# JosephCatrambone/aruco3

Hardware: AMD Instinct MI355X
Metric: frames/sec at 1920x1080 ARUCO dict (higher is better)
Workload: dtype u8

## Files before the change

aruco3_amd/_lib.py:

```python
import ctypes as C
from pathlib import Path

import numpy as np

import os

_HERE = Path(__file__).resolve().parent
LIB_PATH = Path(os.environ["A3_HIP_LIB"]).resolve() if os.environ.get("A3_HIP_LIB") else _HERE / "libaruco3_hip.so"

OK, ERR_INVALID, ERR_HIP, ERR_CAPACITY, ERR_INTERNAL, ERR_NO_DEVICE, ERR_LIMIT = 0, -1, -2, -3, -4, -5, -6
FMT_RGB8, FMT_RGBA8, FMT_L8, FMT_BGRA8 = 0, 1, 2, 3
MEM_HOST, MEM_DEVICE = 0, 1
PROFILE_OFF, PROFILE_STAGES, PROFILE_THRESHOLD_ONLY, PROFILE_THRESHOLD_SAMPLED = 0, 1, 2, 3
STAGE_THRESHOLD, STAGE_CONTOUR, STAGE_DECODE = 0, 1, 2
STEP_WHOLE, STEP_DECODE_DEFERRED, STEP_HELD_RELEASED_BY_LAST, STEP_HELD_RELEASED_EARLY, STEP_BURST_LAST, STEP_HELD = 0, 1, 2, 3, 4, 5
REFINE_NONE, REFINE_SUBPIX = 0, 1
BOARD_NONE, BOARD_OK = 0, 1
BOARD_MAX_MARKERS = 1024
DIST_NONE, DIST_RATIONAL = 0, 1
CHARUCO_MAX_CORNERS = 2048
CHARUCO_NO_ADJ = 0xFFFFFFFF
CALIB_FIX_PRINCIPAL_POINT, CALIB_ZERO_TANGENT_DIST, CALIB_FIX_K3, CALIB_RATIONAL_MODEL, CALIB_USE_INTRINSIC_GUESS = 1, 2, 4, 8, 16
CALIB_OK, CALIB_TOO_FEW, CALIB_NO_INIT, CALIB_NOT_FINITE = 1, 2, 3, 4
CALIB_VIEW_USED, CALIB_VIEW_TOO_FEW_POINTS, CALIB_VIEW_DEGENERATE = 1, 2, 3
CALIB_MAX_POINTS, CALIB_MAX_VIEWS, CALIB_MAX_CAMERAS, CALIB_MAX_CALL_VIEWS = 4096, 4096, 1024, 65536
RIG_USE_EXTRINSIC_GUESS, RIG_FIX_EXTRINSICS = 1, 2
RIG_OK, RIG_NOT_CONNECTED, RIG_NOT_FINITE = 1, 2, 3
RIG_OBS_USED, RIG_OBS_TOO_FEW_POINTS, RIG_OBS_DEGENERATE = 1, 2, 3
RIG_FRAME_USED, RIG_FRAME_UNUSED = 1, 2
RIG_MAX_CAMERAS, RIG_MAX_FRAMES, RIG_MAX_RIGS, RIG_MAX_CALL_FRAMES, RIG_MAX_CALL_OBSERVATIONS = 8, 4096, 1024, 65536, 262144
STEP_NAMES = {0: "whole", 1: "decode_deferred", 2: "held_released_by_last", 3: "held_released_early", 4: "burst_last", 5: "held"}

SYMBOLS = [
    "a3_abi_version", "a3_default_config", "a3_create", "a3_destroy", "a3_last_error", "a3_set_stream", "a3_get_stream", "a3_set_pool_limits",
    "a3_get_tau", "a3_order_after", "a3_set_debug_taps", "a3_detect_batch", "a3_detect_batch_pose", "a3_detect_batch_submit", "a3_detect_batch_collect", "a3_detect_batch_pose_submit", "a3_detect_batch_pose_collect",
    "a3_host_alloc", "a3_host_free", "a3_host_register", "a3_host_unregister", "a3_get_stats", "a3_synth_render", "a3_download_grey", "a3_download_thresholded",
    "a3_candidate_count", "a3_download_candidates", "a3_download_homographies", "a3_estimate_pose", "a3_estimate_pose_normalized",
    "a3_find_nearest", "a3_calculate_tau", "a3_set_profiling", "a3_get_profile",
    "a3_contour_count", "a3_download_contours", "a3_detection_record_bytes", "a3_pack_detections",
    "a3_default_refine_config", "a3_set_corner_refinement", "a3_get_refined_corners", "a3_refine_corners",
    "a3_set_board", "a3_get_board_poses", "a3_estimate_board_pose",
    "a3_default_distortion", "a3_set_distortion", "a3_get_undistorted_corners", "a3_undistort_points",
    "a3_default_charuco_config", "a3_set_charuco", "a3_get_charuco_corners", "a3_get_charuco_poses", "a3_interpolate_charuco",
    "a3_calibrate_cameras", "a3_calibrate_rigs",
]
INTERNAL_SYMBOLS = ["a3_debug_set_overlap", "a3_debug_build_flags", "a3_debug_spin", "a3_debug_set_hold", "a3_debug_set_jump_rounds", "a3_debug_launch_threshold", "a3_debug_kernel_time", "a3_selftest_ieee", "a3_debug_clockwise", "a3_debug_rotate_bits", "a3_debug_discard_too_near", "a3_debug_inject_candidates"]


class A3Error(RuntimeError):
    def __init__(self, code, message):
        super().__init__(f"aruco3_hip error {code}: {message}")
        self.code = code


class Config(C.Structure):
    _fields_ = [
        ("threshold_window", C.c_uint32),
        ("contour_simplification_epsilon", C.c_double),
        ("min_side_length_factor", C.c_float),
        ("min_corner_separation_factor", C.c_float),
        ("homography_sample_size", C.c_uint32),
        ("filter_high_bit_errors", C.c_uint8),
    ]


class MarkerRec(C.Structure):
    _fields_ = [
        ("frame", C.c_uint32),
        ("id", C.c_uint32),
# ... 206 lines not shown
    L.a3_download_homographies.argtypes = [vp, C.c_uint32, u8p, u8p, u64p, C.POINTER(C.c_int32), C.c_size_t]
    L.a3_estimate_pose.restype = C.c_int
    L.a3_estimate_pose.argtypes = [vp, u32p, C.c_size_t, C.c_float, C.POINTER(Intrinsics), C.c_uint32, C.c_uint32, C.POINTER(PoseRec)]
    L.a3_estimate_pose_normalized.restype = C.c_int
    L.a3_estimate_pose_normalized.argtypes = [vp, f32p, C.c_size_t, C.c_float, C.POINTER(PoseRec)]
    L.a3_find_nearest.restype = C.c_int
    L.a3_find_nearest.argtypes = [vp, u64p, C.c_size_t, u32p, u8p]
    L.a3_calculate_tau.restype = C.c_int
    L.a3_calculate_tau.argtypes = [C.c_int, u64p, C.c_size_t, u8p]
    L.a3_set_profiling.restype = C.c_int
    L.a3_set_profiling.argtypes = [vp, C.c_int]
    L.a3_get_profile.restype = C.c_int
    L.a3_get_profile.argtypes = [vp, C.c_int, f64p, u64p, C.c_int]
    L.a3_selftest_ieee.restype = C.c_int
    L.a3_selftest_ieee.argtypes = [vp, f64p, f64p, C.c_size_t, f64p, f64p, f32p, f32p]
    L.a3_contour_count.restype = C.c_int
    L.a3_contour_count.argtypes = [vp, C.c_uint32, u32p, u64p]
    L.a3_download_contours.restype = C.c_int
    L.a3_download_contours.argtypes = [vp, C.c_uint32, u32p, u32p, u32p, C.c_size_t, C.c_size_t]
    L.a3_detection_record_bytes.restype = C.c_size_t
    L.a3_detection_record_bytes.argtypes = [C.c_uint32, C.c_int]
    L.a3_pack_detections.restype = C.c_int
    L.a3_pack_detections.argtypes = [vp, C.c_uint32, C.c_uint32, C.c_int, vp, C.c_size_t]
    L.a3_debug_clockwise.restype = C.c_int
    L.a3_debug_clockwise.argtypes = [vp, C.POINTER(C.c_int32), C.c_size_t, C.POINTER(C.c_int32)]
    L.a3_debug_rotate_bits.restype = C.c_int
    L.a3_debug_rotate_bits.argtypes = [vp, u8p, C.c_uint32, C.c_uint32, u8p]
    L.a3_debug_inject_candidates.restype = C.c_int
    L.a3_debug_inject_candidates.argtypes = [vp, u32p, C.c_size_t]
    if hasattr(L, "a3_refine_corners"):
        L.a3_default_refine_config.restype = None
        L.a3_default_refine_config.argtypes = [C.POINTER(RefineConfig)]
        L.a3_set_corner_refinement.restype = C.c_int
        L.a3_set_corner_refinement.argtypes = [vp, C.POINTER(RefineConfig)]
        L.a3_get_refined_corners.restype = C.c_int
        L.a3_get_refined_corners.argtypes = [vp, f32p, C.c_size_t, C.POINTER(C.c_size_t)]
        L.a3_refine_corners.restype = C.c_int
        L.a3_refine_corners.argtypes = [vp, vp, C.c_int, C.c_int, C.c_uint32, C.c_uint32, C.c_size_t, f32p, f32p, C.c_size_t]
    if hasattr(L, "a3_set_board"):
        L.a3_set_board.restype = C.c_int
        L.a3_set_board.argtypes = [vp, u32p, f32p, C.c_size_t]
        L.a3_get_board_poses.restype = C.c_int
        L.a3_get_board_poses.argtypes = [vp, vp, C.c_size_t, C.POINTER(C.c_size_t)]
        L.a3_estimate_board_pose.restype = C.c_int
        L.a3_estimate_board_pose.argtypes = [vp, u32p, f32p, C.c_size_t, C.POINTER(Intrinsics), C.c_uint32, C.c_uint32, C.POINTER(BoardPoseRec)]
    if hasattr(L, "a3_set_distortion"):
# ... 146 lines not shown

    def order_after(self, other: "Context"):
        check(load().a3_order_after(self.handle, other.handle), self.handle)

    def set_debug_taps(self, on: bool):
        check(load().a3_set_debug_taps(self.handle, int(on)), self.handle)

    def set_pool_limits(self, max_darts: int = 0, max_points: int = 0):
        check(load().a3_set_pool_limits(self.handle, max_darts, max_points), self.handle)

    def set_profiling(self, mode):
        check(load().a3_set_profiling(self.handle, int(mode)), self.handle)

    def profile(self, stage: int, reset: bool = False):
        ms, n = C.c_double(), C.c_uint64()
        check(load().a3_get_profile(self.handle, stage, C.byref(ms), C.byref(n), int(reset)), self.handle)
        return float(ms.value), int(n.value)

    def debug_kernel_time(self, kernel: int, dbg: int = 0, reps: int = 5) -> float:
        ms = C.c_float()
        check(load().a3_debug_kernel_time(self.handle, kernel, dbg, reps, C.byref(ms)), self.handle)
        return ms.value

    def stats(self) -> dict:
        s = Stats()
        check(load().a3_get_stats(self.handle, C.byref(s)), self.handle)
        return s.as_dict()

    def detect_batch(self, pixels_ptr: int, memory: int, fmt: int, width: int, height: int, row_stride: int, frame_stride: int, n_frames: int,
                     out_cap: int = 0):
        cap = out_cap or max(64 * n_frames, 64)
        out = np.empty(cap, dtype=MARKER_DTYPE)
        per = np.zeros(max(n_frames, 1), dtype=np.uint32)
        n = C.c_size_t()
        rc = load().a3_detect_batch(self.handle, C.c_void_p(pixels_ptr), memory, fmt, width, height, row_stride, frame_stride, n_frames,
                                    out.ctypes.data_as(C.c_void_p), cap, _p(per, C.c_uint32), C.byref(n))
        check(rc, self.handle)
        return out[: n.value], per[:n_frames]

    def submit(self, pixels_ptr: int, memory: int, fmt: int, width: int, height: int, row_stride: int, frame_stride: int, n_frames: int,
               out_cap: int = 0):
        self._pending = (out_cap or max(64 * n_frames, 64), n_frames)
        check(load().a3_detect_batch_submit(self.handle, C.c_void_p(pixels_ptr), memory, fmt, width, height, row_stride, frame_stride, n_frames,
                                            self._pending[0]), self.handle)

    def collect(self):
# ... 304 lines not shown
```

aruco3_amd/csrc/a3_api.hip:

```cpp
#include <algorithm>
#include <atomic>
#include <cmath>
#include <chrono>
#include <cstddef>
#include <cstdio>
#include <cstring>
#include <mutex>
#include <string>
#include <vector>

#include "a3_common.h"
#include "a3_internal.h"

namespace a3 {
hipError_t launch_grey_threshold(hipStream_t, const uint8_t*, int, size_t, size_t, int, int, uint32_t, uint32_t, uint8_t*, uint64_t*, uint16_t*);
bool threshold_writes_grey_plane(uint32_t radius, const uint8_t* pixels, size_t row_stride, size_t frame_stride, int W);
hipError_t launch_dart_count(hipStream_t, const uint64_t*, int, int, uint32_t, uint32_t, unsigned long long*, uint32_t*, uint64_t, uint32_t*, uint32_t*, void*, size_t);
size_t tile_darts_bytes(uint32_t W, uint32_t H, uint32_t n_frames);
size_t tile_off_offset(uint32_t W, uint32_t H, uint32_t n_frames);
size_t tile_mask_offset_bytes(uint32_t W, uint32_t H, uint32_t n_frames);
hipError_t launch_dart_build(hipStream_t, const uint64_t*, int, int, uint32_t, uint32_t, const uint32_t*, const uint32_t*, uint32_t*, const uint32_t*,
                             uint64_t*, uint32_t*, uint32_t, const uint32_t*, int, const unsigned long long*);
hipError_t launch_zero(hipStream_t, void*, size_t);
size_t entry_state_bytes();
bool finalize_inline(bool frame_entries, bool trust_natural);
size_t fin_state_bytes();
size_t entry_slots(uint32_t);
size_t leader_list_bytes(uint32_t);
hipError_t launch_rank_cycles(hipStream_t, uint32_t, int, const uint64_t*, const uint32_t*,
                              uint32_t*, unsigned int*, void*, void*, void*, uint32_t*, unsigned int*, int, DeviceCounters*, const uint32_t*, int,
                              const uint32_t*, uint32_t*, uint32_t, int, uint32_t, unsigned int*, int);
hipError_t launch_resolve(hipStream_t, const void*, uint32_t, int, const uint64_t*, const uint32_t*, const unsigned int*, uint64_t*, uint64_t*,
                          DeviceCounters*, int, const uint32_t*);
hipError_t launch_select_scatter(hipStream_t, const void*, uint32_t, const uint32_t*, const unsigned int*, const uint32_t*, const uint64_t*,
                                 const uint32_t*, uint32_t, uint32_t,
                                 uint32_t, double, double, ContourRec*, uint32_t*, uint32_t, uint64_t, DeviceCounters*,
                                 const uint64_t*, uint32_t*, const uint32_t*, int, uint32_t*, int, const void*);
hipError_t launch_debug_clockwise(hipStream_t, const int32_t*, uint32_t, int32_t*);
hipError_t launch_unpack_bits(hipStream_t, const uint64_t*, int, int, uint8_t*);
hipError_t launch_contour_quads(hipStream_t, const ContourRec*, const DeviceCounters*, uint32_t, const uint32_t*, double, uint32_t, uint32_t,
                                uint32_t, CandRec*, uint32_t*, unsigned int*, int, uint32_t);
size_t decode_out_bytes();
hipError_t launch_frame_candidates(hipStream_t, const CandRec*, const uint32_t*, uint32_t, uint32_t, float, uint16_t*, uint16_t*, uint32_t*,
                                   uint32_t*, unsigned int*, uint32_t, void*, float*);
uint32_t frame_cand_lds_slots();
// ... 712 lines not shown
    unsigned int* d_leader_count = ctx->scratch_u32 + 16;
    unsigned int* d_dead_count = ctx->scratch_u32 + 48;

    const uint64_t* d_bin = ctx->bin.as<uint64_t>();
    const double image_diag = std::sqrt((double)W * W + (double)H * H);
    const double eps_factor = ctx->cfg.contour_simplification_epsilon;
    const int resolve_iters = ctx->resolve_full_ttl > 0 ? ctx->resolve_iters_hint : 0;
    const int inline_resolve_W = ctx->resolve_full_ttl > 0 ? 0 : (int)W;
    const int keep_all = b.taps ? 1 : 0;
    int rounds_max = 0;
    for (size_t ci = 0; ci < chunks.size(); ci++) {
        const Chunk& c = chunks[ci];
        DeviceCounters* ctr = ctx->counters + ci;
        const uint32_t* fb = ctx->frame_base.as<uint32_t>() + ci * (max_chunk_frames + 1);
        const uint32_t nd = (uint32_t)c.darts;
        if (nd == 0) continue;
        if (ci > 0) {
            A3_HIP(hipMemsetAsync(d_leader_count, 0, 4 * 32, st));
            A3_HIP(hipMemsetAsync(ctx->frame_cursor, 0, (size_t)c.count * 4, st));
        }
        const uint32_t* tile_off = ctx->tile_darts.as<uint32_t>() + tile_off_offset(W, H, n);
        A3_HIP(launch_dart_build(st, d_bin, (int)W, (int)H, c.first, c.count, fb, tile_off, ctx->pix_base.as<uint32_t>(),
                                 ctx->tile_darts.as<uint32_t>(), ctx->d_xy.as<uint64_t>(), ctx->d_succ.as<uint32_t>(), nd, n_live, 0,
                                 reinterpret_cast<const unsigned long long*>(ctx->tile_darts.as<uint8_t>() + tile_mask_offset_bytes(W, H, n))));
        int rounds = 1;
        while ((1ull << rounds) < (uint64_t)c.max_frame_darts && rounds < 31) rounds++;
        rounds += 1;
        rounds = std::min(rounds, ctx->jump_rounds_hint);
        if (const int cap = g_jump_rounds_cap.load(std::memory_order_relaxed); cap > 0 && ctx->jump_rounds_hint < 32) rounds = std::min(rounds, cap);
        rounds_max = std::max(rounds_max, rounds);
        uint32_t* const frame_entries = ctx->entry_global_ttl > 0 ? nullptr : ctx->frame_cursor;
        const bool dense_graph = (uint64_t)nd * 10u >= (uint64_t)c.count * npx;
        unsigned int* const dead_ctr = (keep_all || !dense_graph) ? nullptr : d_dead_count;
        A3_HIP(launch_rank_cycles(st, nd, (int)W, ctx->d_xy.as<uint64_t>(), ctx->d_succ.as<uint32_t>(),
                                  ctx->entry_list.as<uint32_t>(), d_entry_count, ctx->es_a.p, ctx->es_b.p,
                                  ctx->fin.p, ctx->leader_list.as<uint32_t>(), d_leader_count, rounds, ctr, n_live, 0, fb,
                                  frame_entries, c.count, 1, min_edge_length, dead_ctr, inline_resolve_W > 0 ? 1 : 0));
        if (rel_mode == 2) { if (int rc = release_waiting()) return rc; }
        ctx->dbg_nd = nd; ctx->dbg_frames = c.count; ctx->dbg_chunks = (uint32_t)chunks.size();
        A3_HIP(launch_rank_cycles(st, nd, (int)W, ctx->d_xy.as<uint64_t>(), ctx->d_succ.as<uint32_t>(),
                                  ctx->entry_list.as<uint32_t>(), d_entry_count, ctx->es_a.p, ctx->es_b.p,
                                  ctx->fin.p , ctx->leader_list.as<uint32_t>(), d_leader_count, rounds, ctr,
                                  n_live, 0, fb, frame_entries, c.count, 2, min_edge_length, dead_ctr, inline_resolve_W > 0 ? 1 : 0));
        const void* fin = ctx->fin.p;
        A3_HIP(launch_resolve(st, fin, nd, (int)W, ctx->d_xy.as<uint64_t>(), ctx->leader_list.as<uint32_t>(), d_leader_count,
                              ctx->t_cur.as<uint64_t>(), ctx->t_next.as<uint64_t>(), ctr, resolve_iters, n_live));
        A3_HIP(launch_select_scatter(st, fin, nd, ctx->leader_list.as<uint32_t>(), d_leader_count, ctx->d_succ.as<uint32_t>(), ctx->t_cur.as<uint64_t>(), fb,
// ... 666 lines not shown
    if (int rcs_ = need_stream(ctx)) return rcs_;
    hipStream_t st = ctx->stream;
    struct EventPair {
        hipEvent_t e0 = nullptr, e1 = nullptr;
        ~EventPair() { if (e0) (void)hipEventDestroy(e0); if (e1) (void)hipEventDestroy(e1); }
    } evp;
    A3_HIP(hipEventCreate(&evp.e0)); A3_HIP(hipEventCreate(&evp.e1));
    const hipEvent_t e0 = evp.e0, e1 = evp.e1;
    double total = 0.0;
    unsigned int* d_entry_count = ctx->scratch_u32 + 32;
    unsigned int* d_leader_count = ctx->scratch_u32 + 16;
    for (int r = 0; r < reps; r++) {
        A3_HIP(hipMemsetAsync(d_leader_count, 0, 4 * 32, st));
        A3_HIP(hipEventRecord(e0, st));
        if (kernel == 0) {
            A3_HIP(hipMemsetAsync(ctx->frame_darts.p, 0, (size_t)ctx->frames * 8, st));
            A3_HIP(launch_dart_count(st, ctx->bin.as<uint64_t>(), (int)ctx->W, (int)ctx->H, 0, ctx->frames, ctx->frame_darts.as<unsigned long long>(),
                                     ctx->tile_darts.as<uint32_t>(), 0, nullptr, nullptr, nullptr, 0));
        } else if (kernel == 1) {
            A3_HIP(launch_dart_build(st, ctx->bin.as<uint64_t>(), (int)ctx->W, (int)ctx->H, 0, ctx->dbg_frames, ctx->frame_base.as<uint32_t>(),
                                     ctx->tile_darts.as<uint32_t>() + tile_off_offset(ctx->W, ctx->H, ctx->frames), ctx->pix_base.as<uint32_t>(),
                                     ctx->tile_darts.as<uint32_t>(), ctx->d_xy.as<uint64_t>(),
                                     ctx->d_succ.as<uint32_t>(), ctx->dbg_nd, nullptr, dbg ? dbg : 5,
                                     reinterpret_cast<const unsigned long long*>(ctx->tile_darts.as<uint8_t>() + tile_mask_offset_bytes(ctx->W, ctx->H, ctx->frames))));
        } else if (kernel == 2) {
            A3_HIP(launch_rank_cycles(st, ctx->dbg_nd, (int)ctx->W, ctx->d_xy.as<uint64_t>(), ctx->d_succ.as<uint32_t>(),
                                      ctx->entry_list.as<uint32_t>(),
                                      d_entry_count, ctx->es_a.p, ctx->es_b.p, ctx->fin.p,
                                      ctx->leader_list.as<uint32_t>(), d_leader_count, 0, ctx->counters, nullptr, dbg ? dbg : 11, ctx->frame_base.as<uint32_t>(), nullptr, ctx->dbg_frames, 0,
                                      0u, nullptr, 0));
        } else if (kernel == 3 || kernel == 4) {
            if (kernel == 4) {
                const size_t sweep = std::min<size_t>(ctx->pix_base.cap & ~(size_t)15, (size_t)512 << 20);
                if (sweep) A3_HIP(launch_zero(st, ctx->pix_base.p, sweep));
                A3_HIP(hipEventRecord(e0, st));
            }
            A3_HIP(launch_decode(st, ctx->dbg_src, (int)ctx->W, (int)ctx->H, 0, ctx->fin_xy.as<uint16_t>(), ctx->work.as<uint32_t>(), ctx->scratch_u32,
                                 ctx->max_cand, ctx->cfg.homography_sample_size, ctx->mark_size, ctx->cfg.homography_sample_size, ctx->dict.as<uint64_t>(),
                                 ctx->n_codes, ctx->tau, ctx->cfg.filter_high_bit_errors, ctx->proj.p, ctx->wtab.as<float>(), ctx->outs.p, nullptr, 0u, nullptr, 4096,
                                 dbg == 0 ? -1000 : dbg, ctx->frames <= 64u ? 1 : 0));
        } else return fail(ctx, A3_ERR_INVALID, "kernel: 0 dart_count, 1 dart_assign, 2 local_contract, 3 decode, 4 decode on cold frames");
        A3_HIP(hipEventRecord(e1, st));
        A3_HIP(hipStreamSynchronize(st));
        float ms = 0;
        A3_HIP(hipEventElapsedTime(&ms, e0, e1));
        total += ms;
    }
    *avg_ms = (float)(total / reps);
    return A3_OK;
}

int a3_debug_set_overlap(int mode) {
    if (mode < -1 || mode > 2) return A3_ERR_INVALID;
    std::lock_guard<std::mutex> lk(g_defer_mu);
    if (!g_held.empty() || !g_deferred.empty()) return A3_ERR_INVALID;
    g_overlap_force.store(mode, std::memory_order_relaxed);
    return A3_OK;
}

int a3_debug_spin(void* hip_stream, int workgroups, int threads, int usec) {
    if (workgroups < 1 || workgroups > 1024 || threads < 64 || threads > 512 || threads % 64 || usec < 1 || usec > 100000) return A3_ERR_INVALID;
    static uint32_t* sink = nullptr;
    static std::mutex mu;
    {
        std::lock_guard<std::mutex> lk(mu);
        if (!sink) {
            if (hipMalloc(&sink, 4096 * 4) != hipSuccess) return A3_ERR_HIP;
            if (hipMemset(sink, 0, 4096 * 4) != hipSuccess) return A3_ERR_HIP;
        }
    }
    return launch_spin(reinterpret_cast<hipStream_t>(hip_stream), workgroups, threads, usec, sink) == hipSuccess ? A3_OK : A3_ERR_HIP;
// ... 903 lines not shown
```

aruco3_amd/csrc/a3_internal.h:

```cpp
#ifndef ARUCO3_HIP_INTERNAL_H
#define ARUCO3_HIP_INTERNAL_H

#include "../../include/aruco3_hip.h"

#ifdef __cplusplus
extern "C" {
#endif

int  a3_debug_kernel_time(a3_ctx *ctx, int kernel, int dbg, int reps, float *avg_ms);

int  a3_debug_set_overlap(int mode);

int  a3_debug_spin(void *hip_stream, int workgroups, int threads, int usec);

int  a3_debug_set_hold(int on);

int  a3_debug_set_jump_rounds(int rounds);

int  a3_debug_launch_threshold(a3_ctx *ctx, const void *pixels_device, int fmt, uint32_t width, uint32_t height, uint32_t n_frames);

int  a3_debug_build_flags(void);

int  a3_selftest_ieee(a3_ctx *ctx, const double *a, const double *b, size_t n, double *sqrt_a, double *a_div_b,
                      float *sqrtf_a, float *a_divf_b);

int  a3_debug_clockwise(a3_ctx *ctx, const int32_t *quads_xy, size_t n, int32_t *out_xy);
int  a3_debug_rotate_bits(a3_ctx *ctx, const uint8_t *bits, uint32_t n, uint32_t times, uint8_t *out);
int  a3_debug_inject_candidates(a3_ctx *ctx, const uint32_t *quads_xy, size_t n);
int  a3_debug_discard_too_near(a3_ctx *ctx, const uint32_t *quads_xy, size_t n, float min_distance, uint32_t *out_xy, size_t *n_out);

#ifdef __cplusplus
}
// ... 3 lines not shown
```

aruco3_amd/csrc/k_contours.hip:

```cpp
#include <algorithm>

#include "a3_common.h"


namespace a3 {

constexpr int kFinB = 8;
constexpr int kScatB = 1;

struct Nb8 { uint64_t c; uint64_t n[8]; };

__device__ __forceinline__ uint64_t ldw(const uint64_t* __restrict__ img, int wpr, int H, int j, int y) {
    return (y >= 0 && y < H && j >= 0 && j < wpr) ? img[(size_t)y * wpr + j] : 0ull;
}

__device__ __forceinline__ void pdart_words(const Nb8& nb, uint64_t p[8]) {
#pragma unroll
    for (int k = 0; k < 8; k++) {
        uint64_t m = nb.c & nb.n[k] & ~nb.n[(k + 7) & 7];
        if ((k & 1) == 0) m &= ~nb.n[(k + 6) & 7];
        p[k] = m;
    }
}

// ... 289 lines not shown
struct PixLut { uint16_t v[256]; };
constexpr PixLut make_pix_lut() {
    PixLut t{};
    for (uint32_t F = 0; F < 256; F++) {
        const uint32_t rot1 = ((F << 1) | (F >> 7)) & 0xFFu, rot2 = ((F << 2) | (F >> 6)) & 0xFFu;
        const uint32_t P = F & ~rot1 & (0xAAu | ~rot2) & 0xFFu;
        uint32_t kW = 15, kE = 15;
        if (!(F & 1u)) { kW = 0; for (uint32_t b = 0; b < 7; b++) if ((F >> 1) & (1u << b)) { kW = b + 1; break; } }
        if (!(F & 16u)) {
            const uint32_t rr = ((F >> 5) | (F << 3)) & 0xFFu;
            uint32_t first = 0;
            for (uint32_t b = 0; b < 8; b++) if (rr & (1u << b)) { first = b + 1; break; }
            kE = (5 + first - 1) & 7;
        }
        t.v[F] = (uint16_t)(P | (kW << 8) | (kE << 12));
    }
    return t;
}
__device__ __constant__ const PixLut kPixLut = make_pix_lut();

__device__ __forceinline__ int dir_dx(int k) { return (int)((0x1A90u >> (2 * k)) & 3u) - 1; }
__device__ __forceinline__ int dir_dy(int k) { return (int)((0xA901u >> (2 * k)) & 3u) - 1; }

__global__ __launch_bounds__(256) void k_dart_assign(const uint64_t* __restrict__ bits, int W, int H, uint32_t first_frame,
                                                     const uint32_t* __restrict__ frame_base, const uint32_t* __restrict__ tile_off,
                                                     uint32_t* __restrict__ pix_base, const uint32_t* __restrict__ tile_darts,
                                                     uint64_t* __restrict__ d_rec, uint32_t* __restrict__ d_succ,
                                                     const uint32_t* __restrict__ n_live, int dbg,
                                                     const unsigned long long* __restrict__ tile_mask, uint32_t tiles, uint32_t n_frames) {
    __shared__ uint32_t s_wave[4];
    __shared__ uint64_t s_t[kTileRows + 2][kTileWords + 2];
    __shared__ uint64_t s_nodes[256];
    __shared__ uint64_t s_c0[256], s_c1[256], s_c2[256];
    __shared__ uint32_t s_dbase[256];
    __shared__ uint32_t s_mark[512];
    __shared__ uint16_t s_nbk[256];
    __shared__ uint8_t s_wofrank[256], s_rank[256], s_fr[256];
    __shared__ uint32_t s_multi;
    __shared__ uint16_t s_lut[256];
    const int wpr = (int)words_per_row((uint32_t)W);
    const uint32_t n_wg = tiles * n_frames, chunk = (n_wg + 7u) >> 3, g = (blockIdx.x & 7u) * chunk + (blockIdx.x >> 3);
    if (g >= n_wg) return;
    const uint32_t f = g / tiles, tile = g - f * tiles;
    if (tile_darts[(size_t)(first_frame + f) * tiles + tile] == 0u) return;
    if (n_live && *n_live == 0u) return;
    const uint32_t dart0 = frame_base[f] + tile_off[(size_t)(first_frame + f) * tiles + tile];
    if (dbg == 1) return;
    __shared__ uint32_t s_cnt[256];
    const unsigned long long* tm = tile_mask + ((size_t)(first_frame + f) * tiles + tile) * kCountHalves;
    static_assert(kCountHalves == 4 && kTileWords == 4 && kTileRows == 64, "four 64-bit word masks per tile, four word columns of 64 rows");
    unsigned long long cm[4];
#pragma unroll
    for (int c = 0; c < 4; c++)
        cm[c] = ((tm[0] >> (16 * c)) & 0xFFFFull) | (((tm[1] >> (16 * c)) & 0xFFFFull) << 16) | (((tm[2] >> (16 * c)) & 0xFFFFull) << 32) | (((tm[3] >> (16 * c)) & 0xFFFFull) << 48);
    const unsigned long long m0 = cm[0], m1 = cm[1], m2 = cm[2], m3 = cm[3];
    tile_stage(bits + (size_t)(first_frame + f) * wpr * H, W, H, tile, s_t);
    s_cnt[threadIdx.x] = 0;
    s_mark[threadIdx.x] = 0; s_mark[256 + threadIdx.x] = 0;
    s_lut[threadIdx.x] = kPixLut.v[threadIdx.x];
    if (threadIdx.x == 0) s_multi = 0;
    __syncthreads();
    const uint32_t a0 = (uint32_t)__popcll(m0), a1 = a0 + (uint32_t)__popcll(m1), a2 = a1 + (uint32_t)__popcll(m2), n_act = a2 + (uint32_t)__popcll(m3);
    for (uint32_t k = threadIdx.x; k < n_act; k += 256) {
        const uint32_t part = (k >= a0) + (k >= a1) + (k >= a2);
        const unsigned long long mm = part == 0 ? m0 : (part == 1 ? m1 : (part == 2 ? m2 : m3));
        const uint32_t w = part * 64u + (uint32_t)select_bit(mm, k - (part == 0 ? 0u : (part == 1 ? a0 : (part == 2 ? a1 : a2))));
        const Nb8 nb = tile_nb8(s_t, (int)(w & 63u), (int)(w >> 6));
        uint64_t p[8];
        pdart_words(nb, p);
        uint64_t nodes = 0;
        uint32_t nd = 0;
#pragma unroll
        for (int q = 0; q < 8; q++) { nd += __popcll(p[q]); nodes |= p[q]; }
        const uint64_t s1 = p[0] ^ p[1] ^ p[2], k1 = (p[0] & p[1]) | (p[2] & (p[0] ^ p[1]));
        const uint64_t s2 = p[3] ^ p[4] ^ p[5], k2 = (p[3] & p[4]) | (p[5] & (p[3] ^ p[4]));
        const uint64_t s3 = p[6] ^ p[7], k3 = p[6] & p[7];
        const uint64_t k4 = (s1 & s2) | (s3 & (s1 ^ s2));
        const uint64_t t = k1 ^ k2 ^ k3, q1 = (k1 & k2) | (k3 & (k1 ^ k2));
        s_nodes[w] = nodes;
        const uint64_t c1 = t ^ k4, c2 = q1 | (t & k4);
        s_c0[w] = s1 ^ s2 ^ s3; s_c1[w] = c1; s_c2[w] = c2;
        if ((c1 | c2) != 0ull) s_multi = 1u;
        s_cnt[w] = nd | ((uint32_t)__popcll(nodes) << 17);
        s_wofrank[k] = (uint8_t)w; s_rank[w] = (uint8_t)k;
    }
    __syncthreads();
    uint32_t total_p;
    const uint32_t excl_p = block_excl_scan_256(s_cnt[threadIdx.x], s_wave, &total_p);
    const uint32_t excl_d = excl_p & 0x1FFFFu, excl_n = excl_p >> 17, total_n = total_p >> 17;
    s_dbase[threadIdx.x] = excl_d;
    {
        const uint32_t cw = s_cnt[threadIdx.x] >> 17;
        if (cw) {
            const uint32_t k = s_rank[threadIdx.x];
            s_nbk[k] = (uint16_t)excl_n;
            if (excl_n) atomicOr(&s_mark[(excl_n - 1u) >> 5], 1u << ((excl_n - 1u) & 31u));
            const uint32_t seg = (excl_n + 63u) >> 6;
            if ((seg << 6) < excl_n + cw) s_fr[seg] = (uint8_t)k;
        }
    }
    if (dbg == 2) return;
    __syncthreads();
    if (dbg == 3) return;
    const int tx = tile % dart_tiles_x((uint32_t)W), ty = tile / dart_tiles_x((uint32_t)W);
    uint32_t* pbf = pix_base + (size_t)f * W * H;
    const bool single = __builtin_amdgcn_readfirstlane((int)s_multi) == 0;
    for (uint32_t n = threadIdx.x; n < total_n; n += 256) {
        const uint32_t seg = n >> 6;
        const uint32_t marks_below = __builtin_amdgcn_mbcnt_hi(s_mark[2u * seg + 1u], __builtin_amdgcn_mbcnt_lo(s_mark[2u * seg], 0u));
        const uint32_t kr = (uint32_t)s_fr[seg] + marks_below;
        const uint32_t w = s_wofrank[kr], r = n - (uint32_t)s_nbk[kr];
        const uint64_t m = s_nodes[w];
        const int i = select_bit(m, r);
        const int jl = w >> 6, rl = w & 63;
        const int wj = tx * kTileWords + jl, wy = ty * kTileRows + rl;
        const uint32_t F = tile_F(s_t, rl, jl, i);
        const uint32_t lut = s_lut[F];
        uint32_t P = lut & 0xFFu;
        const uint64_t below = (1ull << i) - 1ull;
        const uint32_t off = single ? (uint32_t)__popcll(m & below)
                                    : (uint32_t)__popcll(s_c0[w] & below) + 2u * (uint32_t)__popcll(s_c1[w] & below) + 4u * (uint32_t)__popcll(s_c2[w] & below);
        const int x = 64 * wj + i;
        uint32_t cur = dart0 + s_dbase[w] + off;
        if ((i == 0 || i == 63 || rl == 0 || rl == kTileRows - 1) && dbg != 4) pbf[(size_t)wy * W + x] = cur;
        const int kW = x > 0 ? (int)((lut >> 8) & 15u) : 15, kE = x + 1 < W ? (int)(lut >> 12) : 15;
        const uint32_t xy = (uint32_t)x | ((uint32_t)wy << 16);
        while (P) {
            const int k = __ffs(P) - 1;
            P &= P - 1;
            const uint32_t info = (uint32_t)k | (k == kW ? kInfoW : 0u) | (k == kE ? kInfoE : 0u);
            if (dbg != 4) d_rec[cur] = dart_rec(xy, F, info, f);
            const uint32_t rr = ((F >> k) | (F << (8 - k))) & 0xFFu;
            const int ko = (k + (31 - __clz(rr))) & 7, kin = (ko + 4) & 7;
            const int lx = jl * 64 + i + dir_dx(ko), ly = rl + dir_dy(ko);
            uint32_t succ;
            if (lx >= 0 && lx < kTileWords * 64 && ly >= 0 && ly < kTileRows) {
                const int j2 = lx >> 6, i2 = lx & 63, w2 = j2 * kTileRows + ly;
                const uint32_t P2 = (uint32_t)s_lut[tile_F(s_t, ly, j2, i2)] & 0xFFu;
                succ = cur;
                if ((P2 >> kin) & 1u) {
                    const uint64_t below2 = (1ull << i2) - 1ull;
                    const uint32_t off2 = single ? (uint32_t)__popcll(s_nodes[w2] & below2)
                                                 : (uint32_t)__popcll(s_c0[w2] & below2) + 2u * (uint32_t)__popcll(s_c1[w2] & below2) +
                                                   4u * (uint32_t)__popcll(s_c2[w2] & below2);
                    succ = dart0 + s_dbase[w2] + off2 + (uint32_t)__popc(P2 & ((1u << kin) - 1u));
                }
            } else {
                succ = kNone;
            }
            if (dbg != 4 || succ == 0x12345678u) d_succ[cur] = succ;
            cur++;
        }
    }
}

__device__ __forceinline__ uint32_t pixel_F(const uint64_t* __restrict__ img, int wpr, int H, int x, int y) {
    const int j = x >> 6, i = x & 63;
    uint32_t rows[3];
#pragma unroll
    for (int dy = -1; dy <= 1; dy++) {
        const uint64_t c = ldw(img, wpr, H, j, y + dy);
        const uint64_t l = i == 0 ? ldw(img, wpr, H, j - 1, y + dy) : 0ull;
        const uint64_t r = i == 63 ? ldw(img, wpr, H, j + 1, y + dy) : 0ull;
        rows[dy + 1] = row3(l, c, r, i);
    }
    const uint32_t top = rows[0], mid = rows[1], bot = rows[2];
    return (mid & 1u) | ((top & 7u) << 1) | ((mid & 4u) << 2) | ((bot & 4u) << 3) | ((bot & 2u) << 5) | ((bot & 1u) << 7);
}

__device__ __forceinline__ uint32_t cross_tile_succ(uint32_t d, uint64_t rec, int W, int H, int wpr, uint32_t first_frame,
                                                    const uint32_t* __restrict__ pix_base, const uint64_t* __restrict__ bits) {
    const uint32_t f = rec_frame(rec);
    const uint64_t* img = bits + (size_t)(first_frame + f) * wpr * H;
    const uint32_t* pb = pix_base + (size_t)f * W * H;
// ... 1030 lines not shown
size_t tile_off_offset(uint32_t W, uint32_t H, uint32_t n_frames) { return (size_t)dart_tiles(W, H) * n_frames; }
size_t tile_mask_offset_bytes(uint32_t W, uint32_t H, uint32_t n_frames) { return ((size_t)dart_tiles(W, H) * n_frames * 4 * (1 + kCountHalves) + 7) & ~(size_t)7; }

hipError_t launch_dart_count(hipStream_t st, const uint64_t* bits, int W, int H, uint32_t first_frame, uint32_t n_frames,
                             unsigned long long* frame_darts, uint32_t* tile_darts, uint64_t plan_cap, uint32_t* frame_base, uint32_t* plan,
                             void* zero_p, size_t zero_bytes ) {
    const uint32_t tiles_x = dart_tiles_x((uint32_t)W), tiles_y = ((uint32_t)H + kTileRows - 1) / kTileRows;
    const uint32_t wpr = words_per_row((uint32_t)W);
    uint32_t* h1 = tile_darts + (size_t)tiles_x * tiles_y * n_frames * 2;
    unsigned long long* tmask = reinterpret_cast<unsigned long long*>(reinterpret_cast<uint8_t*>(tile_darts) + tile_mask_offset_bytes((uint32_t)W, (uint32_t)H, n_frames));
    if (wpr <= 30)
        hipLaunchKernelGGL(k_dart_count<32>, dim3((tiles_y + 1) / 2, n_frames, kCountHalves), dim3(64), 0, st, bits, W, H, first_frame, frame_darts, tile_darts, h1, tmask);
    else
        hipLaunchKernelGGL(k_dart_count<64>, dim3(((wpr + kCountLanes - 1) / kCountLanes) * tiles_y, n_frames, kCountHalves), dim3(64), 0, st, bits, W, H, first_frame,
                           frame_darts, tile_darts, h1, tmask);
    hipLaunchKernelGGL(k_tile_scan, dim3(n_frames + (plan ? 1u : 0u)), dim3(256), 0, st, tile_darts, h1, tiles_x * tiles_y, first_frame,
                       tile_darts + (size_t)tiles_x * tiles_y * n_frames, n_frames, frame_darts, (unsigned long long)plan_cap, frame_base, plan,
                       reinterpret_cast<uint4*>(zero_p), (uint32_t)(zero_bytes / 16));
    return hipGetLastError();
}

hipError_t launch_dart_build(hipStream_t st, const uint64_t* bits, int W, int H, uint32_t first_frame, uint32_t n_frames,
                             const uint32_t* frame_base, const uint32_t* tile_off, uint32_t* pix_base, const uint32_t* tile_darts, uint64_t* d_rec,
                             uint32_t* d_succ, uint32_t n_darts, const uint32_t* n_live, int dbg, const unsigned long long* tile_mask) {
    const uint32_t tiles = dart_tiles((uint32_t)W, (uint32_t)H);
    hipLaunchKernelGGL(k_dart_assign, dim3((tiles * n_frames + 7u) / 8u * 8u), dim3(256), 0, st, bits, W, H, first_frame, frame_base, tile_off,
                       pix_base, tile_darts, d_rec, d_succ, n_live, dbg, tile_mask, tiles, n_frames);
    if (dbg && dbg != 5) return hipGetLastError();
    hipLaunchKernelGGL(k_dart_link, dim3(blocks_for(n_darts, 256, 4096)), dim3(256), 0, st, W, H, first_frame, pix_base, bits, d_rec, d_succ, n_darts, n_live);
    return hipGetLastError();
}

size_t entry_state_bytes() { return sizeof(EntryState); }
bool finalize_inline(bool frame_entries, bool trust_natural) { return frame_entries && trust_natural; }
size_t fin_state_bytes() { return sizeof(FinState); }
size_t entry_slots(uint32_t n_darts) { return (size_t)entry_shard_cap(n_darts) * kEntryShards; }
size_t leader_list_bytes(uint32_t n_darts) { return (size_t)leader_shard_cap(n_darts) * kLeaderShards * 4; }

hipError_t launch_rank_cycles(hipStream_t st, uint32_t n_darts, int W, const uint64_t* d_rec, const uint32_t* d_succ,
                              uint32_t* entry_list,
                              unsigned int* entry_count, void* es_a, void* es_b, void* fin8 , uint32_t* leader_list,
                              unsigned int* leader_count, int max_rounds, DeviceCounters* ctr, const uint32_t* n_live, int dbg,
                              const uint32_t* frame_base, uint32_t* frame_entries , uint32_t n_frames,
                              int phase ,
                              uint32_t min_edge_length, unsigned int* dead_count ,
                              int trust_natural ) {
    const uint32_t ecap = entry_shard_cap(n_darts);
    FinState* fin = reinterpret_cast<FinState*>(fin8);
    const bool no_finalize = finalize_inline(frame_entries != nullptr, trust_natural != 0) && dbg == 0;
    uint32_t* const ll = no_finalize ? leader_list : nullptr;
// ... 95 lines not shown
```

Before: 387,200.

## Add shared-memory pixel table to dart assignment for cheaper successor lookup

```diff
diff --git a/aruco3_amd/_lib.py b/aruco3_amd/_lib.py
--- a/aruco3_amd/_lib.py
+++ b/aruco3_amd/_lib.py
@@ -44,7 +44,7 @@
     "a3_default_charuco_config", "a3_set_charuco", "a3_get_charuco_corners", "a3_get_charuco_poses", "a3_interpolate_charuco",
     "a3_calibrate_cameras", "a3_calibrate_rigs",
 ]
-INTERNAL_SYMBOLS = ["a3_debug_set_overlap", "a3_debug_build_flags", "a3_debug_spin", "a3_debug_set_hold", "a3_debug_set_jump_rounds", "a3_debug_launch_threshold", "a3_debug_kernel_time", "a3_selftest_ieee", "a3_debug_clockwise", "a3_debug_rotate_bits", "a3_debug_discard_too_near", "a3_debug_inject_candidates"]
+INTERNAL_SYMBOLS = ["a3_debug_set_overlap", "a3_debug_build_flags", "a3_debug_spin", "a3_debug_set_hold", "a3_debug_set_jump_rounds", "a3_debug_launch_threshold", "a3_debug_kernel_time", "a3_selftest_ieee", "a3_debug_clockwise", "a3_debug_rotate_bits", "a3_debug_discard_too_near", "a3_debug_inject_candidates", "a3_debug_assign_paths"]
 
 
 class A3Error(RuntimeError):
@@ -297,6 +297,9 @@
     L.a3_detection_record_bytes.argtypes = [C.c_uint32, C.c_int]
     L.a3_pack_detections.restype = C.c_int
     L.a3_pack_detections.argtypes = [vp, C.c_uint32, C.c_uint32, C.c_int, vp, C.c_size_t]
+    if hasattr(L, "a3_debug_assign_paths"):
+        L.a3_debug_assign_paths.restype = C.c_int
+        L.a3_debug_assign_paths.argtypes = [vp, C.POINTER(C.c_uint32)]
     L.a3_debug_clockwise.restype = C.c_int
     L.a3_debug_clockwise.argtypes = [vp, C.POINTER(C.c_int32), C.c_size_t, C.POINTER(C.c_int32)]
     L.a3_debug_rotate_bits.restype = C.c_int
@@ -489,6 +492,11 @@
         check(load().a3_debug_kernel_time(self.handle, kernel, dbg, reps, C.byref(ms)), self.handle)
         return ms.value
 
+    def debug_assign_paths(self):
+        t = (C.c_uint32 * 2)()
+        check(load().a3_debug_assign_paths(self.handle, t), self.handle)
+        return int(t[0]), int(t[1])
+
     def stats(self) -> dict:
         s = Stats()
         check(load().a3_get_stats(self.handle, C.byref(s)), self.handle)
diff --git a/aruco3_amd/csrc/a3_api.hip b/aruco3_amd/csrc/a3_api.hip
--- a/aruco3_amd/csrc/a3_api.hip
+++ b/aruco3_amd/csrc/a3_api.hip
@@ -20,7 +20,7 @@
 size_t tile_off_offset(uint32_t W, uint32_t H, uint32_t n_frames);
 size_t tile_mask_offset_bytes(uint32_t W, uint32_t H, uint32_t n_frames);
 hipError_t launch_dart_build(hipStream_t, const uint64_t*, int, int, uint32_t, uint32_t, const uint32_t*, const uint32_t*, uint32_t*, const uint32_t*,
-                             uint64_t*, uint32_t*, uint32_t, const uint32_t*, int, const unsigned long long*);
+                             uint64_t*, uint32_t*, uint32_t, const uint32_t*, int, const unsigned long long*, unsigned int*);
 hipError_t launch_zero(hipStream_t, void*, size_t);
 size_t entry_state_bytes();
 bool finalize_inline(bool frame_entries, bool trust_natural);
@@ -779,7 +779,7 @@
         const uint32_t* tile_off = ctx->tile_darts.as<uint32_t>() + tile_off_offset(W, H, n);
         A3_HIP(launch_dart_build(st, d_bin, (int)W, (int)H, c.first, c.count, fb, tile_off, ctx->pix_base.as<uint32_t>(),
                                  ctx->tile_darts.as<uint32_t>(), ctx->d_xy.as<uint64_t>(), ctx->d_succ.as<uint32_t>(), nd, n_live, 0,
-                                 reinterpret_cast<const unsigned long long*>(ctx->tile_darts.as<uint8_t>() + tile_mask_offset_bytes(W, H, n))));
+                                 reinterpret_cast<const unsigned long long*>(ctx->tile_darts.as<uint8_t>() + tile_mask_offset_bytes(W, H, n)), nullptr));
         int rounds = 1;
         while ((1ull << rounds) < (uint64_t)c.max_frame_darts && rounds < 31) rounds++;
         rounds += 1;
@@ -1492,7 +1492,7 @@
                                      ctx->tile_darts.as<uint32_t>() + tile_off_offset(ctx->W, ctx->H, ctx->frames), ctx->pix_base.as<uint32_t>(),
                                      ctx->tile_darts.as<uint32_t>(), ctx->d_xy.as<uint64_t>(),
                                      ctx->d_succ.as<uint32_t>(), ctx->dbg_nd, nullptr, dbg ? dbg : 5,
-                                     reinterpret_cast<const unsigned long long*>(ctx->tile_darts.as<uint8_t>() + tile_mask_offset_bytes(ctx->W, ctx->H, ctx->frames))));
+                                     reinterpret_cast<const unsigned long long*>(ctx->tile_darts.as<uint8_t>() + tile_mask_offset_bytes(ctx->W, ctx->H, ctx->frames)), nullptr));
         } else if (kernel == 2) {
             A3_HIP(launch_rank_cycles(st, ctx->dbg_nd, (int)ctx->W, ctx->d_xy.as<uint64_t>(), ctx->d_succ.as<uint32_t>(),
                                       ctx->entry_list.as<uint32_t>(),
@@ -1517,6 +1517,30 @@
         total += ms;
     }
     *avg_ms = (float)(total / reps);
+    return A3_OK;
+}
+
+int a3_debug_assign_paths(a3_ctx* ctx, uint32_t* tiles) {
+    if (!ctx || !tiles) return A3_ERR_INVALID;
+    if (ctx->dbg_chunks != 1 || ctx->dbg_nd == 0) return fail(ctx, A3_ERR_INVALID, "needs a preceding single-chunk batch");
+    A3_HIP(hipSetDevice(ctx->device));
+    if (int rcs_ = need_stream(ctx)) return rcs_;
+    hipStream_t st = ctx->stream;
+    struct Counters {
+        unsigned int* p = nullptr;
+        ~Counters() { if (p) (void)hipFree(p); }
+    } cnt;
+    A3_HIP(hipMalloc(&cnt.p, 2 * sizeof(unsigned int)));
+    A3_HIP(hipMemsetAsync(cnt.p, 0, 2 * sizeof(unsigned int), st));
+    A3_HIP(launch_dart_build(st, ctx->bin.as<uint64_t>(), (int)ctx->W, (int)ctx->H, 0, ctx->dbg_frames, ctx->frame_base.as<uint32_t>(),
+                             ctx->tile_darts.as<uint32_t>() + tile_off_offset(ctx->W, ctx->H, ctx->frames), ctx->pix_base.as<uint32_t>(),
+                             ctx->tile_darts.as<uint32_t>(), ctx->d_xy.as<uint64_t>(), ctx->d_succ.as<uint32_t>(), ctx->dbg_nd, nullptr, 5,
+                             reinterpret_cast<const unsigned long long*>(ctx->tile_darts.as<uint8_t>() + tile_mask_offset_bytes(ctx->W, ctx->H, ctx->frames)),
+                             cnt.p));
+    unsigned int h[2] = {0, 0};
+    A3_HIP(hipMemcpyAsync(h, cnt.p, sizeof(h), hipMemcpyDeviceToHost, st));
+    A3_HIP(hipStreamSynchronize(st));
+    tiles[0] = h[0]; tiles[1] = h[1];
     return A3_OK;
 }
 
diff --git a/aruco3_amd/csrc/a3_internal.h b/aruco3_amd/csrc/a3_internal.h
--- a/aruco3_amd/csrc/a3_internal.h
+++ b/aruco3_amd/csrc/a3_internal.h
@@ -8,6 +8,8 @@
 #endif
 
 int  a3_debug_kernel_time(a3_ctx *ctx, int kernel, int dbg, int reps, float *avg_ms);
+
+int  a3_debug_assign_paths(a3_ctx *ctx, uint32_t tiles[2]);
 
 int  a3_debug_set_overlap(int mode);
 
diff --git a/aruco3_amd/csrc/k_contours.hip b/aruco3_amd/csrc/k_contours.hip
--- a/aruco3_amd/csrc/k_contours.hip
+++ b/aruco3_amd/csrc/k_contours.hip
@@ -1,4 +1,5 @@
 #include <algorithm>
+#include <type_traits>
 
 #include "a3_common.h"
 
@@ -335,22 +336,25 @@
 __device__ __forceinline__ int dir_dx(int k) { return (int)((0x1A90u >> (2 * k)) & 3u) - 1; }
 __device__ __forceinline__ int dir_dy(int k) { return (int)((0xA901u >> (2 * k)) & 3u) - 1; }
 
+constexpr uint32_t kPxCap = 1024;
+
 __global__ __launch_bounds__(256) void k_dart_assign(const uint64_t* __restrict__ bits, int W, int H, uint32_t first_frame,
                                                      const uint32_t* __restrict__ frame_base, const uint32_t* __restrict__ tile_off,
                                                      uint32_t* __restrict__ pix_base, const uint32_t* __restrict__ tile_darts,
                                                      uint64_t* __restrict__ d_rec, uint32_t* __restrict__ d_succ,
                                                      const uint32_t* __restrict__ n_live, int dbg,
-                                                     const unsigned long long* __restrict__ tile_mask, uint32_t tiles, uint32_t n_frames) {
+                                                     const unsigned long long* __restrict__ tile_mask, uint32_t tiles, uint32_t n_frames,
+                                                     unsigned int* __restrict__ path_count) {
     __shared__ uint32_t s_wave[4];
     __shared__ uint64_t s_t[kTileRows + 2][kTileWords + 2];
     __shared__ uint64_t s_nodes[256];
     __shared__ uint64_t s_c0[256], s_c1[256], s_c2[256];
-    __shared__ uint32_t s_dbase[256];
     __shared__ uint32_t s_mark[512];
     __shared__ uint16_t s_nbk[256];
     __shared__ uint8_t s_wofrank[256], s_rank[256], s_fr[256];
     __shared__ uint32_t s_multi;
     __shared__ uint16_t s_lut[256];
+    __shared__ uint32_t s_px[kPxCap];
     const int wpr = (int)words_per_row((uint32_t)W);
     const uint32_t n_wg = tiles * n_frames, chunk = (n_wg + 7u) >> 3, g = (blockIdx.x & 7u) * chunk + (blockIdx.x >> 3);
     if (g >= n_wg) return;
@@ -368,6 +372,7 @@
         cm[c] = ((tm[0] >> (16 * c)) & 0xFFFFull) | (((tm[1] >> (16 * c)) & 0xFFFFull) << 16) | (((tm[2] >> (16 * c)) & 0xFFFFull) << 32) | (((tm[3] >> (16 * c)) & 0xFFFFull) << 48);
     const unsigned long long m0 = cm[0], m1 = cm[1], m2 = cm[2], m3 = cm[3];
     tile_stage(bits + (size_t)(first_frame + f) * wpr * H, W, H, tile, s_t);
+    s_nodes[threadIdx.x] = 0ull;
     s_cnt[threadIdx.x] = 0;
     s_mark[threadIdx.x] = 0; s_mark[256 + threadIdx.x] = 0;
     s_lut[threadIdx.x] = kPixLut.v[threadIdx.x];
@@ -399,11 +404,12 @@
     }
     __syncthreads();
     uint32_t total_p;
-    const uint32_t excl_p = block_excl_scan_256(s_cnt[threadIdx.x], s_wave, &total_p);
-    const uint32_t excl_d = excl_p & 0x1FFFFu, excl_n = excl_p >> 17, total_n = total_p >> 17;
-    s_dbase[threadIdx.x] = excl_d;
+    const uint32_t cnt_w = s_cnt[threadIdx.x];
+    const uint32_t excl_p = block_excl_scan_256(cnt_w, s_wave, &total_p);
+    const uint32_t excl_n = excl_p >> 17, total_n = total_p >> 17;
+    s_cnt[threadIdx.x] = excl_p;
     {
-        const uint32_t cw = s_cnt[threadIdx.x] >> 17;
+        const uint32_t cw = cnt_w >> 17;
         if (cw) {
             const uint32_t k = s_rank[threadIdx.x];
             s_nbk[k] = (uint16_t)excl_n;
@@ -418,23 +424,32 @@
     const int tx = tile % dart_tiles_x((uint32_t)W), ty = tile / dart_tiles_x((uint32_t)W);
     uint32_t* pbf = pix_base + (size_t)f * W * H;
     const bool single = __builtin_amdgcn_readfirstlane((int)s_multi) == 0;
-    for (uint32_t n = threadIdx.x; n < total_n; n += 256) {
+    const bool table = total_n <= kPxCap;
+    if (path_count && threadIdx.x == 0) atomicAdd(&path_count[table ? 0 : 1], 1u);
+    auto locate = [&](uint32_t n, uint32_t& w, int& i, uint64_t& m) {
         const uint32_t seg = n >> 6;
         const uint32_t marks_below = __builtin_amdgcn_mbcnt_hi(s_mark[2u * seg + 1u], __builtin_amdgcn_mbcnt_lo(s_mark[2u * seg], 0u));
         const uint32_t kr = (uint32_t)s_fr[seg] + marks_below;
-        const uint32_t w = s_wofrank[kr], r = n - (uint32_t)s_nbk[kr];
-        const uint64_t m = s_nodes[w];
-        const int i = select_bit(m, r);
+        w = s_wofrank[kr];
+        m = s_nodes[w];
+        i = select_bit(m, n - (uint32_t)s_nbk[kr]);
+    };
+    auto emit = [&](auto kTable, const bool sgl, uint32_t n, uint32_t w, int i, uint32_t F, uint64_t m ) {
+        constexpr bool kTab = decltype(kTable)::value;
         const int jl = w >> 6, rl = w & 63;
         const int wj = tx * kTileWords + jl, wy = ty * kTileRows + rl;
-        const uint32_t F = tile_F(s_t, rl, jl, i);
         const uint32_t lut = s_lut[F];
         uint32_t P = lut & 0xFFu;
-        const uint64_t below = (1ull << i) - 1ull;
-        const uint32_t off = single ? (uint32_t)__popcll(m & below)
-                                    : (uint32_t)__popcll(s_c0[w] & below) + 2u * (uint32_t)__popcll(s_c1[w] & below) + 4u * (uint32_t)__popcll(s_c2[w] & below);
         const int x = 64 * wj + i;
-        uint32_t cur = dart0 + s_dbase[w] + off;
+        uint32_t cur;
+        if (kTab && sgl) {
+            cur = dart0 + n;
+        } else {
+            const uint64_t below = (1ull << i) - 1ull;
+            const uint32_t off = sgl ? (uint32_t)__popcll(m & below)
+                                     : (uint32_t)__popcll(s_c0[w] & below) + 2u * (uint32_t)__popcll(s_c1[w] & below) + 4u * (uint32_t)__popcll(s_c2[w] & below);
+            cur = dart0 + (s_cnt[w] & 0x1FFFFu) + off;
+        }
         if ((i == 0 || i == 63 || rl == 0 || rl == kTileRows - 1) && dbg != 4) pbf[(size_t)wy * W + x] = cur;
         const int kW = x > 0 ? (int)((lut >> 8) & 15u) : 15, kE = x + 1 < W ? (int)(lut >> 12) : 15;
         const uint32_t xy = (uint32_t)x | ((uint32_t)wy << 16);
@@ -449,20 +464,63 @@
             uint32_t succ;
             if (lx >= 0 && lx < kTileWords * 64 && ly >= 0 && ly < kTileRows) {
                 const int j2 = lx >> 6, i2 = lx & 63, w2 = j2 * kTileRows + ly;
-                const uint32_t P2 = (uint32_t)s_lut[tile_F(s_t, ly, j2, i2)] & 0xFFu;
+                const uint64_t below2 = (1ull << i2) - 1ull;
                 succ = cur;
-                if ((P2 >> kin) & 1u) {
-                    const uint64_t below2 = (1ull << i2) - 1ull;
-                    const uint32_t off2 = single ? (uint32_t)__popcll(s_nodes[w2] & below2)
-                                                 : (uint32_t)__popcll(s_c0[w2] & below2) + 2u * (uint32_t)__popcll(s_c1[w2] & below2) +
-                                                   4u * (uint32_t)__popcll(s_c2[w2] & below2);
-                    succ = dart0 + s_dbase[w2] + off2 + (uint32_t)__popc(P2 & ((1u << kin) - 1u));
+                if constexpr (kTab) {
+                    const uint64_t nodes2 = s_nodes[w2];
+                    if ((nodes2 >> i2) & 1ull) {
+                        const uint32_t pre2 = s_cnt[w2];
+                        const uint32_t n2 = (pre2 >> 17) + (uint32_t)__popcll(nodes2 & below2);
+                        const uint32_t P2 = (uint32_t)s_lut[s_px[n2] & 0xFFu] & 0xFFu;
+                        if ((P2 >> kin) & 1u) {
+                            if (sgl) {
+                                succ = dart0 + n2;
+                            } else {
+                                const uint32_t off2 = (uint32_t)__popcll(s_c0[w2] & below2) + 2u * (uint32_t)__popcll(s_c1[w2] & below2) +
+                                                      4u * (uint32_t)__popcll(s_c2[w2] & below2);
+                                succ = dart0 + (pre2 & 0x1FFFFu) + off2 + (uint32_t)__popc(P2 & ((1u << kin) - 1u));
+                            }
+                        }
+                    }
+                } else {
+                    const uint32_t P2 = (uint32_t)s_lut[tile_F(s_t, ly, j2, i2)] & 0xFFu;
+                    if ((P2 >> kin) & 1u) {
+                        const uint32_t off2 = sgl ? (uint32_t)__popcll(s_nodes[w2] & below2)
+                                                  : (uint32_t)__popcll(s_c0[w2] & below2) + 2u * (uint32_t)__popcll(s_c1[w2] & below2) +
+                                                    4u * (uint32_t)__popcll(s_c2[w2] & below2);
+                        succ = dart0 + (s_cnt[w2] & 0x1FFFFu) + off2 + (uint32_t)__popc(P2 & ((1u << kin) - 1u));
+                    }
                 }
             } else {
                 succ = kNone;
             }
             if (dbg != 4 || succ == 0x12345678u) d_succ[cur] = succ;
             cur++;
+        }
+    };
+    if (table) {
+        for (uint32_t n = threadIdx.x; n < total_n; n += 256) {
+            uint32_t w; int i; uint64_t m;
+            locate(n, w, i, m);
+            s_px[n] = tile_F(s_t, (int)(w & 63u), (int)(w >> 6), i) | ((uint32_t)i << 8) | (w << 14);
+        }
+        __syncthreads();
+        if (single) {
+            for (uint32_t n = threadIdx.x; n < total_n; n += 256) {
+                const uint32_t px = s_px[n];
+                emit(std::true_type{}, true, n, px >> 14, (int)((px >> 8) & 63u), px & 0xFFu, 0ull);
+            }
+        } else {
+            for (uint32_t n = threadIdx.x; n < total_n; n += 256) {
+                const uint32_t px = s_px[n];
+                emit(std::true_type{}, false, n, px >> 14, (int)((px >> 8) & 63u), px & 0xFFu, 0ull);
+            }
+        }
+    } else {
+        for (uint32_t n = threadIdx.x; n < total_n; n += 256) {
+            uint32_t w; int i; uint64_t m;
+            locate(n, w, i, m);
+            emit(std::false_type{}, single, n, w, i, tile_F(s_t, (int)(w & 63u), (int)(w >> 6), i), m);
         }
     }
 }
@@ -1539,10 +1597,11 @@
 
 hipError_t launch_dart_build(hipStream_t st, const uint64_t* bits, int W, int H, uint32_t first_frame, uint32_t n_frames,
                              const uint32_t* frame_base, const uint32_t* tile_off, uint32_t* pix_base, const uint32_t* tile_darts, uint64_t* d_rec,
-                             uint32_t* d_succ, uint32_t n_darts, const uint32_t* n_live, int dbg, const unsigned long long* tile_mask) {
+                             uint32_t* d_succ, uint32_t n_darts, const uint32_t* n_live, int dbg, const unsigned long long* tile_mask,
+                             unsigned int* path_count ) {
     const uint32_t tiles = dart_tiles((uint32_t)W, (uint32_t)H);
     hipLaunchKernelGGL(k_dart_assign, dim3((tiles * n_frames + 7u) / 8u * 8u), dim3(256), 0, st, bits, W, H, first_frame, frame_base, tile_off,
-                       pix_base, tile_darts, d_rec, d_succ, n_live, dbg, tile_mask, tiles, n_frames);
+                       pix_base, tile_darts, d_rec, d_succ, n_live, dbg, tile_mask, tiles, n_frames, path_count);
     if (dbg && dbg != 5) return hipGetLastError();
     hipLaunchKernelGGL(k_dart_link, dim3(blocks_for(n_darts, 256, 4096)), dim3(256), 0, st, W, H, first_frame, pix_base, bits, d_rec, d_succ, n_darts, n_live);
     return hipGetLastError();
```

New measurement: 382,900. 1.1% lower.
